# dselivanov/rsparse

Measured on AMD Instinct MI355X. Metric: als_iterations_per_sec, higher is better.
Workload: dtype f32 (Gram products of rows > 512 / <= 32 non-zeros as 2 x fp16 / 3 x bf16 split terms of the fp32 operands, fp32 accumulate; everything else fp32); 1 GPU; WRMF implicit ALS, CG(3), synthetic 10000000x1000000, 500155883 nnz, rank 128, lambda 0.1; survey_config=3, feedback=implicit, n_items=1000000, nnz=500155883, rank=128, solver=conjugate_gradient, cg_steps=3, parallelism=rows sharded x1, factors replicated

## Files before the change

rsparse_amd/build.py:

```python
import subprocess
import sys
import time
from concurrent.futures import ThreadPoolExecutor
from pathlib import Path

PKG = Path(__file__).resolve().parent
CSRC = PKG / "csrc"
SRC = [CSRC / n for n in ("wrmf_kernels.hip", "wrmf_cgq.hip", "wrmf_cgp.hip", "wrmf_ne.hip", "wrmf_chol.hip", "wrmf_chol_wave.hip", "wrmf_chol_mf.hip", "wrmf_cg_mf.hip", "wrmf_chol_lr.hip",
                          "wrmf_topk.hip", "wrmf_topk_large.hip", "wrmf_similar.hip", "wrmf_metrics.hip", "wrmf_hits.hip", "wrmf_lists.hip", "wrmf_diversity.hip", "wrmf_mmr.hip", "wrmf_ranks.hip", "wrmf_score.hip", "wrmf_candidates.hip", "wrmf_sample.hip", "wrmf_sample_weighted.hip", "wrmf_split.hip", "wrmf_explain.hip", "wrmf_init.hip", "wrmf_ingest.hip", "wrmf_nnls.hip", "wrmf_bias.hip", "wrmf_lu.hip",
                          "wrmf_f64.hip", "wrmf_wide.hip", "wrmf_wide_cg.hip", "wrmf_ctx_kernels.hip", "wrmf_schedule.cpp", "wrmf_capi.cpp", "wrmf_f64_capi.cpp", "wrmf_ctx.cpp")]
HEADERS = [CSRC / "wrmf_chol_mf.attrs.csv", CSRC / "wrmf_mf.h", CSRC / "wrmf_internal.h", CSRC / "wrmf_capi_common.h", CSRC / "wrmf_schedule.h", CSRC / "wrmf_device.h", CSRC / "wrmf_sample_team.h", CSRC / "wrmf_wave.h", CSRC / "wrmf_ldlt.h", CSRC / "wrmf_f64.h", PKG.parent / "include" / "rsparse_wrmf_hip.h"]
DEPS = SRC + HEADERS
OUT = PKG / "lib" / "librsparse_wrmf_hip.so"
FLAGS = ["--offload-arch=gfx950", "-O3", "-std=c++17", "-fPIC"]


EXTRA_FLAGS = {n: ["-mllvm", "-forceattrs-csv-path=" + str(CSRC / "wrmf_chol_mf.attrs.csv"), "-fno-slp-vectorize"] for n in ("wrmf_chol_mf.hip", "wrmf_cg_mf.hip")}
AUDITED = {"wrmf_chol_mf.hip", "wrmf_cg_mf.hip"}
REG_LIMIT = {"wrmf_cg_mf.hip": 512}
NO_SPILL = {"wrmf_cgq.hip": ("14als_cgq_kernelILi128ELi24ELi4ELi4E",),
            "wrmf_explain.hip": ("14explain_kernelIfLi128E",),
            "wrmf_sample.hip": ("13sample_kernelILi64E", "13sample_kernelILi256E"),
            "wrmf_sample_weighted.hip": ("22sample_weighted_kernelILi64E", "22sample_weighted_kernelILi256E"),
            "wrmf_hits.hip": ("18hit_metrics_kernelILb0E", "18hit_metrics_kernelILb1E"),
            "wrmf_lists.hip": ("19list_metrics_kernelILb0E", "19list_metrics_kernelILb1E"),
            "wrmf_diversity.hip": ("21list_diversity_kernelI", "21item_inv_norms_kernelI"),
            "wrmf_mmr.hip": ("10mmr_kernelI",),
            "wrmf_split.hip": ("split_count_wave_kernel", "split_count_team_kernel", "split_write_wave_kernel", "split_write_team_kernel")}
RESOURCE_FLAG = "-Rpass-analysis=kernel-resource-usage"


def resource_violations(remarks, patterns, limit=256):
    import re
    rows, cur = [], None
    for line in remarks.splitlines():
# ... 104 lines not shown
```

rsparse_amd/csrc/wrmf_capi.cpp:

```cpp
#include "../../include/rsparse_wrmf_hip.h"

#include <cxxabi.h>

#include <algorithm>
#include <cfloat>
#include <cmath>
#include <cstdlib>
#include <cstring>
#include <string>
#include <vector>

#include "wrmf_capi_common.h"

using namespace rsparse_hip;

struct rsparse_hip_csc {
  DevCSC d;
  int device = 0;
  std::vector<void*> owned;
};

namespace {
thread_local std::string g_err;
}
// ... 272 lines not shown
    if (we != hipSuccess) return hip_fail(we, wave_cg ? "launch_wide_cg_wave" : "launch_als_wide");
    if ((we = launch_sum_partials(g_ws.partials, wave_cg ? (size_t)grid_w : (size_t)grid, outw, s, g_ws.partials + g_ws.partial_slots())) != hipSuccess)
      return hip_fail(we, "launch_sum_partials");
    return RSPARSE_HIP_OK;
  }
  const bool cg = solver == RSPARSE_SOLVER_CONJUGATE_GRADIENT;
  const bool cgq = cg && use_cgq(rank, d_X, d_Y);
  QSchedule qs;
  qs.order = d.q_order;
  qs.cfg = d.q_cfg;
  qs.pair_first = d.q_pair_first;
  for (int b = 0; b < 7; b++) qs.off[b] = d.q_off[b];
  qs.team4_first = (implicit && bias && bias->gbias != 0.f) ? d.q_off[2] : d.q_team4_first;
  qs.team4_wide_first = (implicit && bias && bias->gbias != 0.f) ? d.q_off[2] : d.q_team4_wide_first;
  qs.pair_wide = cgp_wide_supported(rank, implicit, implicit && bias && bias->gbias != 0.f);
  const bool cg_mf = cgq && implicit && !bias && cg_mf_supported(rank, implicit) && d.q_order && d.q_off[1] > d.q_n_nec;
  if (cg_mf) {
    qs.mf_rows = d.q_order + d.q_n_nec;
    qs.mf_n = d.q_off[1] - d.q_n_nec;
  }
  const bool chol_mf = chol_mf_supported(rank) && !cg && solver == RSPARSE_SOLVER_CHOLESKY && !bias && d.q_order && ne_supported(rank) &&
                       use_cgq(rank, d_X, d_Y) && d.q_lr_first > d.q_off[1];
  const int mf_first = d.q_off[1];
  const int n_mf = chol_mf ? d.q_lr_first - mf_first : 0;
  const bool nec_lists = padded_rank(rank) > 64 && d.q_nec.wg > 0 && !chol_mf;
  const bool ne_chol = !cg && solver == RSPARSE_SOLVER_CHOLESKY && !bias && (nec_lists || d.q_ne.wg > 0 || chol_mf) &&
                       ne_supported(rank) && use_cgq(rank, d_X, d_Y);
  qs.ne = (cg_mf || (ne_chol && nec_lists)) ? d.q_nec : ((implicit && padded_rank(rank) == 128) ? d.q_ne : d.q_ne1);
  const size_t chol_base = chol2_loss_slots(d.n_cols);
  const size_t slots = cgq ? cgq_loss_slots(qs, rank, implicit) : (cg ? cg_loss_slots(d.n_cols, d.n_long)
// ... 1896 lines not shown
```

rsparse_amd/csrc/wrmf_cgp.hip:

```cpp
#include "wrmf_internal.h"
#include "wrmf_device.h"

namespace rsparse_hip {
namespace {

using namespace dev;

constexpr int kPairMaxSweeps = 4;

template <int NQ>
struct PairSmem {
  static constexpr int KP = 128, ps = KP + 8, os = KP + 4;
  static constexpr size_t gfrag = NQ == 16 ? (size_t)4 * 16 * 1024 : 0;
  static constexpr size_t nxt = NQ == 16 ? (size_t)4 * 2 * 2 * 64 * 4 : 0;
  static constexpr size_t bytes = gfrag + (size_t)2 * 8 * ps * 2 + (size_t)8 * os * 4 + (size_t)4 * 8 * NQ * 4 + nxt + 16;
};

template <bool GB, bool KFULL = false, int NQ = 8>
__global__ __launch_bounds__(256, 2) void als_cgp_kernel(AlsArgs a, const int32_t* __restrict__ rows, int n_rows, int iters,
                                                        size_t loss_slot0) {
  constexpr int KP = 128, RPN = 8, VW = 4, NV = 2;
  static_assert(NQ == 8 || (NQ == 16 && KFULL && !GB), "the 32-slot kernel: rank 128, no global bias");
  constexpr bool GREG = NQ == 8;
  using SM = PairSmem<NQ>;
  extern __shared__ __attribute__((aligned(16))) char smem[];
  char* sGf = smem + (size_t)(threadIdx.x >> 6) * 16 * 1024;
  _Float16* sPh = reinterpret_cast<_Float16*>(smem + SM::gfrag);
  _Float16* sPl = sPh + 8 * SM::ps;
  float* sOut = reinterpret_cast<float*>(sPl + 8 * SM::ps);
  float* sTsv = sOut + 8 * SM::os;
  float* sNx = sTsv + 4 * 8 * NQ + (threadIdx.x >> 6) * 256;
  const int tid = threadIdx.x, lane = tid & 63, wv = rfl(tid >> 6);
  const int g = lane >> 4, i = lane & 15, H = lane >> 5, g2 = g & 1;
  const int k = KFULL ? KP : a.k;
  const float gbias = GB ? a.gbias : 0.f, ltgt = GB ? a.loss_tgt_const : 1.f;
  for (int e = tid; e < 4 * 8 * NQ; e += 256) sTsv[e] = 0.f;
  f16x8 gAh[GREG ? 2 : 1][GREG ? 4 : 1], gAl[GREG ? 2 : 1][GREG ? 4 : 1];
  float ginv;
  {
    const int m = lane & 15, kb = lane >> 4;
    float gmax = 0.f;
#pragma unroll
    for (int t = 0; t < 2; t++)
#pragma unroll
      for (int ks = 0; ks < 4; ks++)
#pragma unroll
        for (int e = 0; e < 8; e++) {
          const int r = 32 * wv + 16 * t + m, c = 32 * ks + 8 * kb + e;
// ... 19 lines not shown
          const float g1v = a.XtX[(size_t)min(r, k - 1) * k + min(c + 1, k - 1)];
          const float g1 = g1v * ((r < k && c + 1 < k) ? 1.f : 0.f);
          split_f16(g0 * gs, g1 * gs, hi[e / 2], lo[e / 2]);
        }
        const uint4 h4 = {hi[0], hi[1], hi[2], hi[3]}, l4 = {lo[0], lo[1], lo[2], lo[3]};
        if constexpr (GREG) {
          gAh[t][ks] = __builtin_bit_cast(f16x8, h4);
          gAl[t][ks] = __builtin_bit_cast(f16x8, l4);
        } else {
          *reinterpret_cast<uint4*>(sGf + ((t * 4 + ks) * 2 + 0) * 1024 + lane * 16) = h4;
          *reinterpret_cast<uint4*>(sGf + ((t * 4 + ks) * 2 + 1) * 1024 + lane * 16) = l4;
        }
      }
  }
  __syncthreads();
  float* tacc = sTsv + wv * 8 * NQ + 2 * NQ * H;
  float* tcur = tacc + 4 * NQ;
  const int lslot = NQ == 16 ? i + 16 * g2 : i;
  const bool lgrp = NQ == 16 || g2 == 0;
  const int col = 2 * wv + H;
  double wloss = 0.0;
  const int wave_global = blockIdx.x * 4 + wv, total_waves = gridDim.x * 4;
  auto ridx = [&](const int itn) { return (wave_global + itn * total_waves) * 2 + H; };
  int row_c = 0, p1_c = 0, p2_c = 0, row_n = 0;
  if (iters > 0 && ridx(0) < n_rows) {
    row_c = rows[ridx(0)];
    p1_c = a.col_ptrs[row_c];
    p2_c = a.col_ptrs[row_c + 1];
  }
  if (iters > 1 && ridx(1) < n_rows) row_n = rows[ridx(1)];

  int idn[GREG ? NQ : 1];
  float cvn[GREG ? NQ : 1], cln = 0.f;
#pragma unroll
  for (int q = 0; q < (GREG ? NQ : 1); q++) {
    idn[q] = 0;
    cvn[q] = 0.f;
  }
  auto request_indices = [&](const bool valid, const int np1, const int ncnt, const int buf) {
    if constexpr (!GREG) {
      const int e = lane & 31;
      const bool in = valid && e < ncnt;
      float* slot = sNx + buf * 128;
      dma4(in ? static_cast<const void*>(a.row_idx + np1 + e) : static_cast<const void*>(a.zero_row), (unsigned)rfl((int)lds_addr(slot)));
      dma4(in ? static_cast<const void*>(a.vals + np1 + e) : static_cast<const void*>(a.zero_row), (unsigned)rfl((int)lds_addr(slot + 64)));
      return;
    }
#pragma unroll
    for (int q = 0; q < NQ; q++) {
      const int s = 2 * q + g2;
      const int j = (valid && s < ncnt) ? np1 + s : 0;
      idn[q] = a.row_idx[j];
      cvn[q] = a.vals[j];
    }
    cln = a.vals[(valid && lslot < ncnt) ? np1 + lslot : 0];
  };
// ... 21 lines not shown
      int p1_n = 0, p2_n = 0, row_nn = 0;
      if (it + 1 < iters && ridx(it + 1) < n_rows) {
        p1_n = a.col_ptrs[row_n];
        p2_n = a.col_ptrs[row_n + 1];
      }
      if (it + 2 < iters && ridx(it + 2) < n_rows) row_nn = rows[ridx(it + 2)];
      row_c = row_n;
      p1_c = p1_n;
      p2_c = p2_n;
      row_n = row_nn;
    }
    const int cnt = p2 - p1;
    float* yrow = a.Y + (size_t)row * k;
    const bool live = have && (GB || cnt > 0);
    if (have && !live) {
      for (int e = lane & 31; e < k; e += 32) yrow[e] = 0.f;
    }
    const int wcnt = max(__builtin_amdgcn_readlane(cnt, 0), __builtin_amdgcn_readlane(cnt, 32));
    auto blk_on = [&](const int q) { return q < 4 || wcnt > 2 * (q & ~3); };

    float x[RPN], r[RPN], p[RPN], ap[RPN];
    auto load_warm_start = [&]() {
#pragma unroll
      for (int b = 0; b < NV; b++) {
        const int off = b * 16 * VW + i * VW;
        float4 pc = make_float4(0.f, 0.f, 0.f, 0.f);
        if (have && off < k) pc = *reinterpret_cast<const float4*>(yrow + off);
        const float* pf = reinterpret_cast<const float*>(&pc);
#pragma unroll
        for (int c = 0; c < VW; c++) x[b * VW + c] = pf[c];
      }
    };
    if constexpr (KFULL) load_warm_start();
    float xt[NQ][RPN], cv[GREG ? NQ : 1];
    const float* nx = sNx + (it & 1) * 128 + 32 * H;
    {
      int id[NQ];
#pragma unroll
      for (int q = 0; q < NQ; q++) {
        if constexpr (!GREG) {
          id[q] = __float_as_int(nx[2 * q + g2]);
        } else if constexpr (KFULL) {
          id[q] = idn[q];
          cv[q] = cvn[q];
        } else {
          const int s = 2 * q + g2;
          const int j = s < cnt ? p1 + s : 0;
          id[q] = 0;
          cv[q] = 0.f;
          if (blk_on(q)) {
            id[q] = a.row_idx[j];
            cv[q] = a.vals[j];
          }
        }
      }
#pragma unroll
      for (int q = 0; q < NQ; q++) {
        const bool in = 2 * q + g2 < cnt;
        id[q] = in ? id[q] : 0;
        if constexpr (GREG) cv[q] = in ? cv[q] : 0.f;
      }
#pragma unroll
      for (int q = 0; q < NQ; q++) {
        const bool in = 2 * q + g2 < cnt;
        const float* src = in ? a.X + (size_t)id[q] * k : a.zero_row;
#pragma unroll
        for (int b = 0; b < NV; b++) {
          const int off = b * 16 * VW + i * VW;
          if constexpr (KFULL) {
            float4 pc = make_float4(0.f, 0.f, 0.f, 0.f);
            if (blk_on(q)) pc = *reinterpret_cast<const float4*>(src + off);
            const float* pf = reinterpret_cast<const float*>(&pc);
#pragma unroll
            for (int c = 0; c < VW; c++) xt[q][b * VW + c] = pf[c];
          } else {
            float4 pc = make_float4(0.f, 0.f, 0.f, 0.f);
            if (blk_on(q)) pc = *reinterpret_cast<const float4*>(src + min(off, k - VW));
            const float* pf = reinterpret_cast<const float*>(&pc);
#pragma unroll
// ... 2 lines not shown
        }
      }
    }
    float cl;
    if constexpr (!GREG) cl = nx[64 + lslot];
    else if constexpr (KFULL) cl = (lgrp && lslot < cnt) ? cln : 0.f;
    else cl = (lgrp && lslot < cnt) ? a.vals[p1 + lslot] : 0.f;

    if constexpr (!KFULL) load_warm_start();

    auto sweep = [&](const float(&v)[RPN], const int mode, float(&out)[RPN], float& loss_out) {
      float acc[RPN];
#pragma unroll
      for (int rr = 0; rr < RPN; rr++) acc[rr] = 0.f;
      float vinv = 0.f;
      if (mode != 2) {
        float vmax = 0.f;
#pragma unroll
        for (int rr = 0; rr < RPN; rr++) vmax = fmaxf(vmax, fabsf(v[rr]));
        vmax = row16_max(vmax);
        const int ve = fp16_scale_exp(vmax);
        const float vs = __uint_as_float((unsigned)ve << 23);
        vinv = __uint_as_float((unsigned)(254 - ve) << 23) * (mode == 0 ? -1.f : 1.f);
        {
          float w4[VW];
#pragma unroll
          for (int c = 0; c < VW; c++) w4[c] = (g2 == 0 ? v[c] : v[VW + c]) * vs;
          unsigned h0, l0, h1, l1;
          split_f16(w4[0], w4[1], h0, l0);
          split_f16(w4[2], w4[3], h1, l1);
          const int off = col * SM::ps + g2 * 16 * VW + i * VW;
          *reinterpret_cast<uint2*>(sPh + off) = make_uint2(h0, h1);
          *reinterpret_cast<uint2*>(sPl + off) = make_uint2(l0, l1);
        }
        __syncthreads();
        f32x4 d0[2], d1[2];
#pragma unroll
        for (int t = 0; t < 2; t++) d0[t] = d1[t] = f32x4{0.f, 0.f, 0.f, 0.f};
        const int nb = (lane & 7) * SM::ps + 8 * (lane >> 4);
#pragma unroll
        for (int ks = 0; ks < 4; ks++) {
          const f16x8 bh = *reinterpret_cast<const f16x8*>(sPh + nb + 32 * ks);
          const f16x8 bl = *reinterpret_cast<const f16x8*>(sPl + nb + 32 * ks);
#pragma unroll
          for (int t = 0; t < 2; t++) {
            f16x8 ah, al;
            if constexpr (GREG) {
              ah = gAh[t][ks];
              al = gAl[t][ks];
            } else {
              ah = *reinterpret_cast<const f16x8*>(sGf + ((t * 4 + ks) * 2 + 0) * 1024 + lane * 16);
              al = *reinterpret_cast<const f16x8*>(sGf + ((t * 4 + ks) * 2 + 1) * 1024 + lane * 16);
            }
            d0[t] = __builtin_amdgcn_mfma_f32_16x16x32_f16(ah, bh, d0[t], 0, 0, 0);
            d1[t] = __builtin_amdgcn_mfma_f32_16x16x32_f16(ah, bl, d1[t], 0, 0, 0);
            d1[t] = __builtin_amdgcn_mfma_f32_16x16x32_f16(al, bh, d1[t], 0, 0, 0);
          }
        }
        if ((lane & 15) < 8) {
#pragma unroll
          for (int t = 0; t < 2; t++) {
            const f32x4 d = (d0[t] + d1[t]) * ginv;
            *reinterpret_cast<f32x4*>(sOut + (lane & 15) * SM::os + 32 * wv + 16 * t + 4 * (lane >> 4)) = d;
          }
        }
      }
      float lacc = 0.f;
      if (mode != 2) {
        float* trec = (mode == 0 ? tacc : tcur) + g2;
#pragma unroll
        for (int q0 = 0; q0 < NQ; q0 += 4) {
          if (blk_on(q0)) {
            float t[4];
            f32x2 s2[4];
#pragma unroll
            for (int u = 0; u < 4; u++) s2[u] = f32x2{0.f, 0.f};
#pragma unroll
            for (int rr = 0; rr < RPN; rr += 2) {
              const f32x2 va = {v[rr], v[rr + 1]};
#pragma unroll
              for (int u = 0; u < 4; u++) {
                const f32x2 xa = {xt[q0 + u][rr], xt[q0 + u][rr + 1]};
                s2[u] = __builtin_elementwise_fma(xa, va, s2[u]);
              }
            }
#pragma unroll
            for (int u = 0; u < 4; u++) t[u] = s2[u].x + s2[u].y;
#pragma unroll
            for (int u = 0; u < 4; u++) t[u] += dpp<0xB1>(t[u]);
#pragma unroll
            for (int u = 0; u < 4; u++) t[u] += dpp<0x4E>(t[u]);
#pragma unroll
            for (int u = 0; u < 4; u++) t[u] += dpp<0x141>(t[u]);
#pragma unroll
            for (int u = 0; u < 4; u++) t[u] += dpp<0x140>(t[u]);
#pragma unroll
            for (int u = 0; u < 4; u++) {
              const int q = q0 + u;
              const float c = GREG ? cv[q] : nx[64 + 2 * q + g2];
              trec[2 * q] = t[u];
              const float w = mode == 0 ? c - (c - 1.f) * (GB ? t[u] + gbias : t[u]) : (c - 1.f) * t[u];
#pragma unroll
              for (int rr = 0; rr < RPN; rr++) acc[rr] = fmaf(w, xt[q][rr], acc[rr]);
            }
          }
        }
      } else {
        wave_sync();
        const float t = tacc[lslot];
        const float dd = ltgt - t;
        lacc = pair_sum(row16_sum((lgrp && lslot < cnt) ? cl * dd * dd : 0.f));
      }
      if (mode != 2) {
        __syncthreads();
        const float f = g2 == 0 ? vinv : 0.f;
#pragma unroll
        for (int b = 0; b < NV; b++) {
          const f32x4 o = *reinterpret_cast<const f32x4*>(sOut + col * SM::os + b * 16 * VW + i * VW);
#pragma unroll
          for (int c = 0; c < VW; c++) acc[b * VW + c] = fmaf(f, o[c], acc[b * VW + c]);
        }
#pragma unroll
        for (int rr = 0; rr < RPN; rr++) out[rr] = pair_sum(acc[rr]);
        if constexpr (GB) {
          if (mode == 0) {
#pragma unroll
            for (int b = 0; b < NV; b++) {
              const int off = b * 16 * VW + i * VW;
              const float4 pc = *reinterpret_cast<const float4*>(a.rhs_init + min(off, k - VW));
              const float* pf = reinterpret_cast<const float*>(&pc);
#pragma unroll
              for (int c = 0; c < VW; c++) out[b * VW + c] += off < k ? pf[c] : 0.f;
            }
          }
        }
      } else {
        loss_out = lacc;
      }
// ... 33 lines not shown
          const float beta = (float)((double)rsnew / (double)rsold);
#pragma unroll
          for (int rr = 0; rr < RPN; rr++) p[rr] = fmaf(p[rr], beta, r[rr]);
          rsold = rsnew;
        }
      }
    }
    float rl = 0.f;
    sweep(x, 2, ap, rl);
    if constexpr (KFULL) {
      settle_indices();
    }
    if (live) {
      const float xx = dot16(x, x);
      wloss += (double)rl + a.lambda_loss * (double)xx;
      if (g2 == 0) {
#pragma unroll
        for (int b = 0; b < NV; b++) {
          const int off = b * 16 * VW + i * VW;
          if (off < k) {
            float4 pc;
            float* pf = reinterpret_cast<float*>(&pc);
#pragma unroll
            for (int c = 0; c < VW; c++) pf[c] = x[b * VW + c];
            *reinterpret_cast<float4*>(yrow + off) = pc;
          }
        }
      }
    }
  }
  const double other = __shfl(wloss, 32);
  if (lane == 0) a.loss_partials[loss_slot0 + (size_t)blockIdx.x * 4 + wv] = wloss + other;
}

}

bool cgp_supported(int k, bool implicit) { return implicit && k > 64 && k <= 128 && k % 4 == 0; }
bool cgp_wide_supported(int k, bool implicit, bool gbias) { return implicit && k == 128 && !gbias; }

int cgp_grid(int n_rows) {
  if (n_rows <= 0) return 0;
  const long pairs = ((long)n_rows + 1) / 2;
  long per_wave = 32;
  const long spread = 4L * 512;
  if (pairs < spread * per_wave) per_wave = (pairs + spread - 1) / spread;
  if (per_wave < 1) per_wave = 1;
  return (int)((pairs + 4 * per_wave - 1) / (4 * per_wave));
}

hipError_t launch_als_cgp(const AlsArgs& a, const int32_t* rows, int n_rows, bool wide, size_t loss_slot0, hipStream_t s,
                          hipEvent_t* ev_slot) {
  const int grid = cgp_grid(n_rows);
  if (grid <= 0) return hipSuccess;
  const long pairs = ((long)n_rows + 1) / 2;
  const int iters = (int)((pairs + (long)grid * 4 - 1) / ((long)grid * 4));
  const bool gb = a.gbias != 0.f;
  const bool full = !gb && a.k == 128;
  if (wide && !full) return hipErrorInvalidValue;
  auto k0 = als_cgp_kernel<false, false>;
  auto k0f = als_cgp_kernel<false, true>;
  auto k1 = als_cgp_kernel<true, false>;
  auto kw = als_cgp_kernel<false, true, 16>;
  const void* fn = wide ? reinterpret_cast<const void*>(kw)
                        : gb ? reinterpret_cast<const void*>(k1) : (full ? reinterpret_cast<const void*>(k0f) : reinterpret_cast<const void*>(k0));
  const size_t lds = wide ? PairSmem<16>::bytes : PairSmem<8>::bytes;
  hipError_t err = hipFuncSetAttribute(fn, hipFuncAttributeMaxDynamicSharedMemorySize, (int)lds);
  if (err != hipSuccess) return err;
  prof_note(ev_slot, fn);
  if (wide) hipLaunchKernelGGL(kw, dim3(grid), dim3(256), lds, s, a, rows, n_rows, iters, loss_slot0);
  else if (gb) hipLaunchKernelGGL(k1, dim3(grid), dim3(256), lds, s, a, rows, n_rows, iters, loss_slot0);
  else if (full) hipLaunchKernelGGL(k0f, dim3(grid), dim3(256), lds, s, a, rows, n_rows, iters, loss_slot0);
  else hipLaunchKernelGGL(k0, dim3(grid), dim3(256), lds, s, a, rows, n_rows, iters, loss_slot0);
  return hipGetLastError();
}

}
```

rsparse_amd/csrc/wrmf_cgq.hip:

```cpp
#include <algorithm>

#include "wrmf_internal.h"
#include "wrmf_device.h"

namespace rsparse_hip {
namespace {

using namespace dev;

constexpr int kGvFirstMinCapq = 16;
constexpr int kStreamPrefixQ = 4;
constexpr int kIdxPrefetchMaxWpr = 2;

constexpr int kMaxSavedSweeps = 4;

template <int KP>
struct QG {
  static constexpr int RPN = KP / 16;
  static constexpr int VW = RPN >= 4 ? 4 : RPN;
  static constexpr int NV = RPN / VW;
  __device__ static __forceinline__ int elem(int i, int r) { return (r / VW) * (16 * VW) + i * VW + (r % VW); }
};

template <int VW>
struct Piece;
template <>
struct Piece<4> { using type = float4; };
template <>
struct Piece<2> { using type = float2; };

__device__ __forceinline__ float groups_reduce_scatter4(const float a0, const float a1, const float a2, const float a3) {
  const auto s01 = __builtin_amdgcn_permlane16_swap(__float_as_uint(a0), __float_as_uint(a1), false, false);
  const float c = __uint_as_float(s01[0]) + __uint_as_float(s01[1]);
  const auto s23 = __builtin_amdgcn_permlane16_swap(__float_as_uint(a2), __float_as_uint(a3), false, false);
  const float d = __uint_as_float(s23[0]) + __uint_as_float(s23[1]);
  const auto t = __builtin_amdgcn_permlane32_swap(__float_as_uint(c), __float_as_uint(d), false, false);
  return __uint_as_float(t[0]) + __uint_as_float(t[1]);
}
template <bool ON>
__device__ __forceinline__ int opaque_lane(int l) {
  if constexpr (ON) asm volatile("" : "+v"(l));
  return l;
}
template <int KP, int CAPQ, int WAVES, int WPR, int STREAM, bool IMPLICIT, int DMF = 0>
struct QSmem {
  static constexpr size_t gram_floats = (IMPLICIT && DMF != 1) ? (size_t)KP * KP : 0;
  static constexpr size_t vec_floats = IMPLICIT ? (size_t)WAVES * KP : 0;
  static constexpr size_t red_floats = WPR > 1 ? (size_t)2 * WAVES * KP + 2 * WAVES : 0;
  static constexpr bool cv_lds = !STREAM && CAPQ * (KP / 16) > 128;
  static constexpr bool wideq = !STREAM && CAPQ * (KP / 16) > 160;
  static constexpr size_t tsv_floats = (STREAM && !IMPLICIT) ? 0 : (size_t)WAVES * (cv_lds ? 3 : 2) * CAPQ * 4;
  static constexpr size_t pre_floats = STREAM ? (size_t)WAVES * kStreamPrefixQ * 4 * KP : 0;
  static constexpr int dmf_ps = KP + 8, dmf_os = KP + 4;
  static constexpr size_t dmf_floats = DMF ? (size_t)WAVES * dmf_ps + (size_t)WAVES * dmf_os : 0;
  static constexpr size_t pfx_floats =
      (!STREAM && WPR > kIdxPrefetchMaxWpr && (CAPQ == 16 || CAPQ == 20 || CAPQ == 24)) ? (size_t)WAVES * 2 * CAPQ * 4 : 0;
  static constexpr size_t wl_floats = cv_lds ? (size_t)WAVES * 2 : 0;
// ... 917 lines not shown
int concurrent_buckets() { return g_launch_mode; }

size_t bucket_slots(const QSchedule& q, int b, int k, bool implicit) {
  const int cfg = cfg_of_kp(padded_rank(k));
  const BucketDef d = kBuckets[cfg][b];
  if (d.wpr <= 0) return 0;
  if (d.stream && ne_supported(k)) return (size_t)(q.ne.entries + q.ne.nsplit) + (size_t)(q.mf_n > 0 ? cg_mf_loss_slots(q.mf_n) : 0);
  const int rows = q.off[b + 1] - q.off[b];
  if (b == 1 && padded_rank(k) == 128) {
    const int wide = team4_wide_first(q), split = team4_first(q);
    return (size_t)cgq_bucket_grid(wide - q.off[b], b, cfg) * d.waves + (size_t)cgq_team4_wide_grid(split - wide) * kTeam4Waves +
           (size_t)cgq_team4_grid(q.off[b + 1] - split) * kTeam4Waves;
  }
  if (b == kNB - 1 && rows > 0 && cgp_supported(k, implicit)) {
    const int split = std::min(std::max(q.pair_first, q.off[b]), q.off[b + 1]);
    const size_t main = q.pair_wide ? (size_t)cgp_grid(split - q.off[b]) * 4 : (size_t)cgq_bucket_grid(split - q.off[b], b, cfg) * d.waves;
    return main + (size_t)cgp_grid(q.off[b + 1] - split) * 4;
  }
  return (size_t)cgq_bucket_grid(rows, b, cfg) * d.waves;
}

template <int KP, int CFG, bool IMPLICIT, bool GB>
hipError_t launch_all(const AlsArgs& a, const QSchedule& q, hipStream_t s, hipEvent_t* ev) {
  hipError_t err;
  size_t slot = 0;
  const int cmode = ev ? 0 : concurrent_buckets();
  const bool overlap = cmode != 0;
  bool forked = false;
  if (overlap) {
    if ((err = g_bs.ensure()) != hipSuccess) return err;
  }
#define RSP_BUCKET(B)                                                                                       \
// ... 49 lines not shown
          const int g_main = cgq_bucket_grid(n_main, B, CFG), g_w4 = cgq_team4_wide_grid(n_w4);             \
          if ((err = launch_bucket<KP, D.waves, D.capq, D.wpr, D.stream, IMPLICIT, GB>(a, q.order + first, n_main, g_main, slot, \
                                                                                  bs, ev ? ev + B : nullptr)) != hipSuccess) \
            return err;                                                                                     \
          if ((err = launch_bucket<KP, kTeam4Waves, kTeam4WideCapq, kTeam4Waves, 0, IMPLICIT, GB>(          \
                   a, q.order + wide, n_w4, g_w4, slot + (size_t)g_main * D.waves, bs,                      \
                   n_main > 0 ? nullptr : (ev ? ev + B : nullptr))) != hipSuccess)                          \
            return err;                                                                                     \
          if ((err = launch_bucket<KP, kTeam4Waves, kTeam4Capq, kTeam4Waves, 0, IMPLICIT, GB>(              \
                   a, q.order + split, n_t4, cgq_team4_grid(n_t4),                                          \
                   slot + (size_t)g_main * D.waves + (size_t)g_w4 * kTeam4Waves, bs,                        \
                   n_main + n_w4 > 0 ? nullptr : (ev ? ev + B : nullptr))) != hipSuccess)                   \
            return err;                                                                                     \
        } else if (B == kNB - 1 && cgp_supported(a.k, IMPLICIT)) {                    \
           \
                                                 \
          const int first = q.off[B], split = std::min(std::max(q.pair_first, first), q.off[B + 1]);         \
          const int n_main = split - first, n_pair = q.off[B + 1] - split;                                   \
          size_t main_slots;                                                                                \
          if (q.pair_wide) {                                                                                \
            if ((err = launch_als_cgp(a, q.order + first, n_main, true, slot, bs, ev ? ev + B : nullptr)) != hipSuccess) \
              return err;                                                                                   \
            main_slots = (size_t)cgp_grid(n_main) * 4;                                                      \
          } else {                                                                                          \
            const int g_main = cgq_bucket_grid(n_main, B, CFG);                                             \
            if ((err = launch_bucket<KP, D.waves, D.capq, D.wpr, D.stream, IMPLICIT, GB>(a, q.order + first, n_main, g_main, slot, \
                                                                                    bs, ev ? ev + B : nullptr)) != hipSuccess) \
              return err;                                                                                   \
            main_slots = (size_t)g_main * D.waves;                                                          \
          }                                                                                                 \
          if ((err = launch_als_cgp(a, q.order + split, n_pair, false, slot + main_slots, bs,               \
                                    n_main > 0 ? nullptr : (ev ? ev + B : nullptr))) != hipSuccess)           \
            return err;                                                                                     \
        } else if ((err = launch_bucket<KP, D.waves, D.capq, D.wpr, D.stream, IMPLICIT, GB>(a, q.order + q.off[B], n, grid, slot, \
                                                                                bs, ev ? ev + B : nullptr)) != hipSuccess) \
          return err;                                                                                       \
        if (side) {                                                                                         \
          if ((err = hipEventRecord(g_bs.done[B], bs)) != hipSuccess) return err;                           \
          if ((err = hipStreamWaitEvent(s, g_bs.done[B], 0)) != hipSuccess) return err;                     \
        }                                                                                                   \
      }                                                                                                     \
      slot += bucket_slots(q, B, a.k, IMPLICIT);                                                             \
    }                                                                                                       \
  }
  RSP_BUCKET(0)
  RSP_BUCKET(1)
// ... 73 lines not shown
```

rsparse_amd/csrc/wrmf_internal.h:

```cpp
#pragma once
#include <hip/hip_runtime.h>
#include <cstdint>
#include <string>

#include "wrmf_schedule.h"

namespace rsparse_hip {

constexpr float kCgTol = 1e-10f;
constexpr double kCgTolD = 1e-10;
constexpr int kScdMaxIter = 10000;
constexpr float kScdTol = 1e-4f;
constexpr double kScdTolD = 1e-4;
constexpr float kNnlsEps = 1e-16f;
constexpr double kNnlsEpsD = 1e-16;

struct NeListSet {
  const int32_t* rows = nullptr;
  const int32_t* ptr = nullptr;
  int wg = 0;
  int entries = 0;
  const int32_t* segs = nullptr;
  int nseg = 0;
  const int32_t* split_rows = nullptr;
// ... 83 lines not shown
  int* ne_seg_flags;
  int ne_chol;
  int ne_chol_min;
  const unsigned* ne_stats;
  const float* mf_XtX;
  const unsigned* wave_stats;
};

struct QSchedule {
  const int32_t* order;
  int off[7];
  int pair_first;
  int team4_first;
  int team4_wide_first;
  bool pair_wide;
  int cfg;
  NeListSet ne;
  const int32_t* mf_rows = nullptr;
  int mf_n = 0;
};
int cgq_default_cfg();
void cgq_set_launch_mode(int mode);
int cgq_num_buckets();
int cgq_bucket_wpr(int cfg, int b);
int cgq_bucket_capq(int cfg, int b);
int cgq_bucket_waves(int cfg, int b);
int cgq_bucket_stream(int cfg, int b);
int cgq_bucket_grid(int n_rows, int bucket, int cfg);
int cgq_team4_grid(int n_rows);
int cgq_team4_wide_grid(int n_rows);
int cgq_bucket_of(int len, int cfg);
size_t cgq_loss_slots(const QSchedule& q, int k, bool implicit);
bool cgp_supported(int k, bool implicit);
bool cgp_wide_supported(int k, bool implicit, bool gbias);
int cgp_grid(int n_rows);
hipError_t launch_als_cgp(const AlsArgs& a, const int32_t* rows, int n_rows, bool wide, size_t loss_slot0, hipStream_t s,
                          hipEvent_t* ev_slot);
bool ne_supported(int k);
constexpr int kNeMinLen = 512;
constexpr int kNeSegFloats = 4 * (11 * 16 * 64 + 128 + 2);
hipError_t launch_ne_stats(const float* X, int64_t nx, const float* vals, int64_t nnz, unsigned* stats, hipStream_t s,
                           const float* absmax_hint = nullptr, const unsigned* cached_vstats = nullptr,
                           unsigned* save_vstats = nullptr);
hipError_t launch_als_ne(const AlsArgs& a, const QSchedule& q, bool implicit, double* row_loss, hipStream_t s,
                         hipEvent_t* ev_slot = nullptr);
hipError_t launch_gb_row_terms(const AlsArgs& a, const int32_t* rows, int n, float* out, int32_t* slot_of_row, hipStream_t s);
hipError_t launch_als_cgq(const AlsArgs& a, const QSchedule& q, bool implicit, hipStream_t s, hipEvent_t* ev = nullptr);

constexpr int kWavesPerWG = 4;
constexpr int kRowsPerWGShort = 64;
constexpr int kRowsPerWGLong = 8;
// ... 265 lines not shown
```

rsparse_amd/csrc/wrmf_schedule.cpp:

```cpp
#include "wrmf_schedule.h"

#include <algorithm>
#include <functional>
#include <queue>
#include <utility>

namespace rsparse_hip {

namespace {
int ne_slots(int cus) { return 2 * std::max(cus, 1); }
}

NeCut ne_cut(const int32_t* order, const int32_t* col_ptrs, int n_prefix, int64_t fixed, int cus) {
  NeCut c;
  if (n_prefix <= 0) return c;
  auto len_of = [&](int r) { return (int64_t)(col_ptrs[order[r] + 1] - col_ptrs[order[r]]); };
  auto steps_of = [](int64_t len) { return (len + 15) / 16; };
  const int n_slots = ne_slots(cus);
  int64_t total = 0;
  for (int r = 0; r < n_prefix; r++) total += steps_of(len_of(r)) + fixed;
  const int64_t share = std::max<int64_t>(1, total / n_slots);
  c.items.reserve((size_t)n_prefix + 64);
  int n_seg = 0;
  for (int r = 0; r < n_prefix; r++) {
    const int64_t len = len_of(r);
    const int64_t st = steps_of(len);
// ... 110 lines not shown
```

rsparse_amd/csrc/wrmf_schedule.h:

```cpp
#pragma once
#include <cstdint>
#include <vector>

namespace rsparse_hip {

constexpr int kTileNnz = 32;
constexpr int kTeam4Max = 320;
constexpr int kTeam4WideMax = 384;
constexpr int kCholLrMax = 64;
constexpr int kCholLongLen = 4096;
constexpr int kCgMfMax = 16384;
constexpr int kNeMaxSeg = 16;
constexpr int kNeMaxSegTotal = 1024;

struct NeCut {
  struct Item { int64_t cost; int32_t entry; };
  std::vector<Item> items;
  std::vector<int32_t> segs;
  std::vector<int32_t> split_rows;
  std::vector<int32_t> split_ptr;
  int nseg() const { return (int)(segs.size() / 6); }
};
struct NeDeal {
  std::vector<int32_t> rows, ptr;
  int wg() const { return ptr.empty() ? 0 : (int)ptr.size() - 1; }
};

NeCut ne_cut(const int32_t* order, const int32_t* col_ptrs, int n_prefix, int64_t fixed, int cus);
// ... 27 lines not shown
```

rsparse_amd/csrc/wrmf_wave.h:

```cpp
#pragma once
#include <hip/hip_runtime.h>

#include <type_traits>
#include <utility>

namespace rsparse_hip {
namespace dev {

typedef unsigned long long u64;
typedef float f32x2 __attribute__((ext_vector_type(2)));
typedef float f32x4 __attribute__((ext_vector_type(4)));
typedef float f32x16 __attribute__((ext_vector_type(16)));
typedef double f64x4 __attribute__((ext_vector_type(4)));
typedef _Float16 f16x2 __attribute__((ext_vector_type(2)));
typedef _Float16 f16x8 __attribute__((ext_vector_type(8)));
typedef __bf16 bf16x2 __attribute__((ext_vector_type(2)));
typedef __bf16 bf16x8 __attribute__((ext_vector_type(8)));
typedef unsigned u32x4 __attribute__((ext_vector_type(4)));

template <class F, int... I>
__device__ __forceinline__ void static_for_seq(F&& f, std::integer_sequence<int, I...>) {
  (f(std::integral_constant<int, I>{}), ...);
}
template <int N, class F>
__device__ __forceinline__ void static_for(F&& f) {
  static_for_seq(f, std::make_integer_sequence<int, N>{});
}

__device__ __forceinline__ void wave_sync() {
  __builtin_amdgcn_fence(__ATOMIC_RELEASE, "wavefront");
  __builtin_amdgcn_wave_barrier();
  __builtin_amdgcn_fence(__ATOMIC_ACQUIRE, "wavefront");
}

__device__ __forceinline__ float readlane_f(float v, int l) {
  return __int_as_float(__builtin_amdgcn_readlane(__float_as_int(v), l));
}
__device__ __forceinline__ int rfl(int v) { return __builtin_amdgcn_readfirstlane(v); }

__device__ __forceinline__ unsigned lds_addr(const void* p) {
  return (unsigned)(reinterpret_cast<uintptr_t>(p));
}
__device__ __forceinline__ void dma4(const void* g, unsigned lds_base) {
  asm volatile("s_mov_b32 m0, %1\n\ts_nop 0\n\tglobal_load_lds_dword %0, off" : : "v"(g), "s"(lds_base) : "memory", "m0");
}
__device__ __forceinline__ void dma16(const void* g, unsigned lds_base) {
  asm volatile("s_mov_b32 m0, %1\n\ts_nop 0\n\tglobal_load_lds_dwordx4 %0, off" : : "v"(g), "s"(lds_base) : "memory", "m0");
}
template <int N>
__device__ __forceinline__ void wait_vm() {
  asm volatile("s_waitcnt vmcnt(%0)" ::"n"(N) : "memory");
}

// ... 142 lines not shown
```

Measured before the change: 8.564 iterations/s.

## Add four-rows-per-wave CG pair kernel for short rows at rank 128

Adds a QUAD variant of the pair CG kernel in which each wave handles four short rows (16 lanes each, 16 slots per row) instead of two. The fp16 hi/lo panel and the output buffer share one LDS region, and the scheduler selects this variant for the short-row tail when rank is 128 with no global bias. The grid, visit count and loss-slot math are generalised to rows-per-wave. The aim is to use more of each wave on rows with few non-zeros, at the cost of an extra workgroup barrier and register-held B fragments per CG step.

```diff
diff --git a/rsparse_amd/build.py b/rsparse_amd/build.py
--- a/rsparse_amd/build.py
+++ b/rsparse_amd/build.py
@@ -19,6 +19,7 @@
 AUDITED = {"wrmf_chol_mf.hip", "wrmf_cg_mf.hip"}
 REG_LIMIT = {"wrmf_cg_mf.hip": 512}
 NO_SPILL = {"wrmf_cgq.hip": ("14als_cgq_kernelILi128ELi24ELi4ELi4E",),
+            "wrmf_cgp.hip": ("14als_cgp_kernelILb0ELb1ELi16ELb1E",),
             "wrmf_explain.hip": ("14explain_kernelIfLi128E",),
             "wrmf_sample.hip": ("13sample_kernelILi64E", "13sample_kernelILi256E"),
             "wrmf_sample_weighted.hip": ("22sample_weighted_kernelILi64E", "22sample_weighted_kernelILi256E"),
diff --git a/rsparse_amd/csrc/wrmf_capi.cpp b/rsparse_amd/csrc/wrmf_capi.cpp
--- a/rsparse_amd/csrc/wrmf_capi.cpp
+++ b/rsparse_amd/csrc/wrmf_capi.cpp
@@ -310,6 +310,7 @@
   qs.team4_first = (implicit && bias && bias->gbias != 0.f) ? d.q_off[2] : d.q_team4_first;
   qs.team4_wide_first = (implicit && bias && bias->gbias != 0.f) ? d.q_off[2] : d.q_team4_wide_first;
   qs.pair_wide = cgp_wide_supported(rank, implicit, implicit && bias && bias->gbias != 0.f);
+  qs.pair_quad = cgp_quad_supported(rank, implicit, implicit && bias && bias->gbias != 0.f);
   const bool cg_mf = cgq && implicit && !bias && cg_mf_supported(rank, implicit) && d.q_order && d.q_off[1] > d.q_n_nec;
   if (cg_mf) {
     qs.mf_rows = d.q_order + d.q_n_nec;
diff --git a/rsparse_amd/csrc/wrmf_cgp.hip b/rsparse_amd/csrc/wrmf_cgp.hip
--- a/rsparse_amd/csrc/wrmf_cgp.hip
+++ b/rsparse_amd/csrc/wrmf_cgp.hip
@@ -8,30 +8,40 @@
 
 constexpr int kPairMaxSweeps = 4;
 
-template <int NQ>
+template <int NQ, bool QUAD = false>
 struct PairSmem {
-  static constexpr int KP = 128, ps = KP + 8, os = KP + 4;
+  static constexpr int KP = 128, ps = KP + 8, os = QUAD ? KP + 8 : KP + 4;
+  static constexpr int cols = QUAD ? 16 : 8;
+  static constexpr int pcs = QUAD ? 2 * ps : ps;
   static constexpr size_t gfrag = NQ == 16 ? (size_t)4 * 16 * 1024 : 0;
   static constexpr size_t nxt = NQ == 16 ? (size_t)4 * 2 * 2 * 64 * 4 : 0;
-  static constexpr size_t bytes = gfrag + (size_t)2 * 8 * ps * 2 + (size_t)8 * os * 4 + (size_t)4 * 8 * NQ * 4 + nxt + 16;
+  static constexpr size_t pub = (size_t)2 * cols * ps * 2, out = (size_t)cols * os * 4;
+  static_assert(!QUAD || (pub == out && (size_t)pcs * 2 == (size_t)os * 4), "QUAD: one column, one stretch of LDS");
+  static constexpr size_t bytes = gfrag + (QUAD ? pub : pub + out) + (size_t)4 * 8 * NQ * 4 + nxt + 16;
 };
-
-template <bool GB, bool KFULL = false, int NQ = 8>
+static_assert(PairSmem<16>::bytes <= 81920 && PairSmem<16, true>::bytes <= 81920, "two workgroups per CU");
+
+template <bool GB, bool KFULL = false, int NQ = 8, bool QUAD = false>
 __global__ __launch_bounds__(256, 2) void als_cgp_kernel(AlsArgs a, const int32_t* __restrict__ rows, int n_rows, int iters,
                                                         size_t loss_slot0) {
   constexpr int KP = 128, RPN = 8, VW = 4, NV = 2;
   static_assert(NQ == 8 || (NQ == 16 && KFULL && !GB), "the 32-slot kernel: rank 128, no global bias");
+  static_assert(!QUAD || NQ == 16, "four rows per wave: 16 slots per group, G in LDS");
   constexpr bool GREG = NQ == 8;
-  using SM = PairSmem<NQ>;
+  constexpr int RW = QUAD ? 4 : 2, GL = 64 / RW;
+  constexpr int SS = QUAD ? 1 : 2;
+  using SM = PairSmem<NQ, QUAD>;
   extern __shared__ __attribute__((aligned(16))) char smem[];
   char* sGf = smem + (size_t)(threadIdx.x >> 6) * 16 * 1024;
   _Float16* sPh = reinterpret_cast<_Float16*>(smem + SM::gfrag);
-  _Float16* sPl = sPh + 8 * SM::ps;
-  float* sOut = reinterpret_cast<float*>(sPl + 8 * SM::ps);
-  float* sTsv = sOut + 8 * SM::os;
+  _Float16* sPl = QUAD ? sPh + SM::ps : sPh + 8 * SM::ps;
+  float* sOut = QUAD ? reinterpret_cast<float*>(sPh) : reinterpret_cast<float*>(sPl + 8 * SM::ps);
+  float* sTsv = QUAD ? reinterpret_cast<float*>(sPh + 16 * SM::pcs) : sOut + 8 * SM::os;
   float* sNx = sTsv + 4 * 8 * NQ + (threadIdx.x >> 6) * 256;
   const int tid = threadIdx.x, lane = tid & 63, wv = rfl(tid >> 6);
   const int g = lane >> 4, i = lane & 15, H = lane >> 5, g2 = g & 1;
+  const int R = QUAD ? g : H;
+  const int gs = QUAD ? 0 : g2;
   const int k = KFULL ? KP : a.k;
   const float gbias = GB ? a.gbias : 0.f, ltgt = GB ? a.loss_tgt_const : 1.f;
   for (int e = tid; e < 4 * 8 * NQ; e += 256) sTsv[e] = 0.f;
@@ -81,14 +91,14 @@
       }
   }
   __syncthreads();
-  float* tacc = sTsv + wv * 8 * NQ + 2 * NQ * H;
+  float* tacc = sTsv + wv * 8 * NQ + (QUAD ? NQ * g : 2 * NQ * H);
   float* tcur = tacc + 4 * NQ;
-  const int lslot = NQ == 16 ? i + 16 * g2 : i;
+  const int lslot = (NQ == 16 && !QUAD) ? i + 16 * g2 : i;
   const bool lgrp = NQ == 16 || g2 == 0;
-  const int col = 2 * wv + H;
+  const int col = RW * wv + R;
   double wloss = 0.0;
   const int wave_global = blockIdx.x * 4 + wv, total_waves = gridDim.x * 4;
-  auto ridx = [&](const int itn) { return (wave_global + itn * total_waves) * 2 + H; };
+  auto ridx = [&](const int itn) { return (wave_global + itn * total_waves) * RW + R; };
   int row_c = 0, p1_c = 0, p2_c = 0, row_n = 0;
   if (iters > 0 && ridx(0) < n_rows) {
     row_c = rows[ridx(0)];
@@ -106,7 +116,7 @@
   }
   auto request_indices = [&](const bool valid, const int np1, const int ncnt, const int buf) {
     if constexpr (!GREG) {
-      const int e = lane & 31;
+      const int e = lane & (GL - 1);
       const bool in = valid && e < ncnt;
       float* slot = sNx + buf * 128;
       dma4(in ? static_cast<const void*>(a.row_idx + np1 + e) : static_cast<const void*>(a.zero_row), (unsigned)rfl((int)lds_addr(slot)));
@@ -158,10 +168,16 @@
     float* yrow = a.Y + (size_t)row * k;
     const bool live = have && (GB || cnt > 0);
     if (have && !live) {
-      for (int e = lane & 31; e < k; e += 32) yrow[e] = 0.f;
-    }
-    const int wcnt = max(__builtin_amdgcn_readlane(cnt, 0), __builtin_amdgcn_readlane(cnt, 32));
-    auto blk_on = [&](const int q) { return q < 4 || wcnt > 2 * (q & ~3); };
+      if constexpr (QUAD) {
+#pragma unroll
+        for (int b = 0; b < NV; b++) *reinterpret_cast<float4*>(yrow + b * 16 * VW + i * VW) = make_float4(0.f, 0.f, 0.f, 0.f);
+      } else {
+        for (int e = lane & 31; e < k; e += 32) yrow[e] = 0.f;
+      }
+    }
+    int wcnt = max(__builtin_amdgcn_readlane(cnt, 0), __builtin_amdgcn_readlane(cnt, 32));
+    if constexpr (QUAD) wcnt = max(wcnt, max(__builtin_amdgcn_readlane(cnt, 16), __builtin_amdgcn_readlane(cnt, 48)));
+    auto blk_on = [&](const int q) { return q < 4 || wcnt > SS * (q & ~3); };
 
     float x[RPN], r[RPN], p[RPN], ap[RPN];
     auto load_warm_start = [&]() {
@@ -177,13 +193,13 @@
     };
     if constexpr (KFULL) load_warm_start();
     float xt[NQ][RPN], cv[GREG ? NQ : 1];
-    const float* nx = sNx + (it & 1) * 128 + 32 * H;
+    const float* nx = sNx + (it & 1) * 128 + (QUAD ? 16 * g : 32 * H);
     {
       int id[NQ];
 #pragma unroll
       for (int q = 0; q < NQ; q++) {
         if constexpr (!GREG) {
-          id[q] = __float_as_int(nx[2 * q + g2]);
+          id[q] = __float_as_int(QUAD ? nx[q] : nx[2 * q + g2]);
         } else if constexpr (KFULL) {
           id[q] = idn[q];
           cv[q] = cvn[q];
@@ -200,13 +216,13 @@
       }
 #pragma unroll
       for (int q = 0; q < NQ; q++) {
-        const bool in = 2 * q + g2 < cnt;
+        const bool in = SS * q + gs < cnt;
         id[q] = in ? id[q] : 0;
         if constexpr (GREG) cv[q] = in ? cv[q] : 0.f;
       }
 #pragma unroll
       for (int q = 0; q < NQ; q++) {
-        const bool in = 2 * q + g2 < cnt;
+        const bool in = SS * q + gs < cnt;
         const float* src = in ? a.X + (size_t)id[q] * k : a.zero_row;
 #pragma unroll
         for (int b = 0; b < NV; b++) {
@@ -239,6 +255,8 @@
 #pragma unroll
       for (int rr = 0; rr < RPN; rr++) acc[rr] = 0.f;
       float vinv = 0.f;
+      const int ln = opaque_lane<QUAD>(lane), li = ln & 15, lg = ln >> 4;
+      const int lcol = QUAD ? RW * wv + lg : col;
       if (mode != 2) {
         float vmax = 0.f;
 #pragma unroll
@@ -247,7 +265,18 @@
         const int ve = fp16_scale_exp(vmax);
         const float vs = __uint_as_float((unsigned)ve << 23);
         vinv = __uint_as_float((unsigned)(254 - ve) << 23) * (mode == 0 ? -1.f : 1.f);
-        {
+        if constexpr (QUAD) {
+          wave_sync();
+#pragma unroll
+          for (int b = 0; b < NV; b++) {
+            unsigned h0, l0, h1, l1;
+            split_f16(v[b * VW] * vs, v[b * VW + 1] * vs, h0, l0);
+            split_f16(v[b * VW + 2] * vs, v[b * VW + 3] * vs, h1, l1);
+            const int off = lcol * SM::pcs + b * 16 * VW + li * VW;
+            *reinterpret_cast<uint2*>(sPh + off) = make_uint2(h0, h1);
+            *reinterpret_cast<uint2*>(sPl + off) = make_uint2(l0, l1);
+          }
+        } else {
           float w4[VW];
 #pragma unroll
           for (int c = 0; c < VW; c++) w4[c] = (g2 == 0 ? v[c] : v[VW + c]) * vs;
@@ -262,11 +291,26 @@
         f32x4 d0[2], d1[2];
 #pragma unroll
         for (int t = 0; t < 2; t++) d0[t] = d1[t] = f32x4{0.f, 0.f, 0.f, 0.f};
-        const int nb = (lane & 7) * SM::ps + 8 * (lane >> 4);
+        const int nb = QUAD ? li * SM::pcs + 8 * lg : (lane & 7) * SM::ps + 8 * (lane >> 4);
+        f16x8 bhs[QUAD ? 4 : 1], bls[QUAD ? 4 : 1];
+        if constexpr (QUAD) {
+#pragma unroll
+          for (int ks = 0; ks < 4; ks++) {
+            bhs[ks] = *reinterpret_cast<const f16x8*>(sPh + nb + 32 * ks);
+            bls[ks] = *reinterpret_cast<const f16x8*>(sPl + nb + 32 * ks);
+          }
+          __syncthreads();
+        }
 #pragma unroll
         for (int ks = 0; ks < 4; ks++) {
-          const f16x8 bh = *reinterpret_cast<const f16x8*>(sPh + nb + 32 * ks);
-          const f16x8 bl = *reinterpret_cast<const f16x8*>(sPl + nb + 32 * ks);
+          f16x8 bh, bl;
+          if constexpr (QUAD) {
+            bh = bhs[ks];
+            bl = bls[ks];
+          } else {
+            bh = *reinterpret_cast<const f16x8*>(sPh + nb + 32 * ks);
+            bl = *reinterpret_cast<const f16x8*>(sPl + nb + 32 * ks);
+          }
 #pragma unroll
           for (int t = 0; t < 2; t++) {
             f16x8 ah, al;
@@ -274,25 +318,26 @@
               ah = gAh[t][ks];
               al = gAl[t][ks];
             } else {
-              ah = *reinterpret_cast<const f16x8*>(sGf + ((t * 4 + ks) * 2 + 0) * 1024 + lane * 16);
-              al = *reinterpret_cast<const f16x8*>(sGf + ((t * 4 + ks) * 2 + 1) * 1024 + lane * 16);
+              ah = *reinterpret_cast<const f16x8*>(sGf + ((t * 4 + ks) * 2 + 0) * 1024 + (QUAD ? ln : lane) * 16);
+              al = *reinterpret_cast<const f16x8*>(sGf + ((t * 4 + ks) * 2 + 1) * 1024 + (QUAD ? ln : lane) * 16);
             }
             d0[t] = __builtin_amdgcn_mfma_f32_16x16x32_f16(ah, bh, d0[t], 0, 0, 0);
             d1[t] = __builtin_amdgcn_mfma_f32_16x16x32_f16(ah, bl, d1[t], 0, 0, 0);
             d1[t] = __builtin_amdgcn_mfma_f32_16x16x32_f16(al, bh, d1[t], 0, 0, 0);
           }
         }
-        if ((lane & 15) < 8) {
+        if (QUAD || (lane & 15) < 8) {
 #pragma unroll
           for (int t = 0; t < 2; t++) {
             const f32x4 d = (d0[t] + d1[t]) * ginv;
-            *reinterpret_cast<f32x4*>(sOut + (lane & 15) * SM::os + 32 * wv + 16 * t + 4 * (lane >> 4)) = d;
+            float* po = QUAD ? sOut + li * SM::os + 32 * wv + 16 * t + 4 * lg : sOut + (lane & 15) * SM::os + 32 * wv + 16 * t + 4 * (lane >> 4);
+            *reinterpret_cast<f32x4*>(po) = d;
           }
         }
       }
       float lacc = 0.f;
       if (mode != 2) {
-        float* trec = (mode == 0 ? tacc : tcur) + g2;
+        float* trec = (mode == 0 ? tacc : tcur) + gs;
 #pragma unroll
         for (int q0 = 0; q0 < NQ; q0 += 4) {
           if (blk_on(q0)) {
@@ -322,8 +367,8 @@
 #pragma unroll
             for (int u = 0; u < 4; u++) {
               const int q = q0 + u;
-              const float c = GREG ? cv[q] : nx[64 + 2 * q + g2];
-              trec[2 * q] = t[u];
+              const float c = GREG ? cv[q] : (QUAD ? nx[64 + q] : nx[64 + 2 * q + g2]);
+              trec[SS * q] = t[u];
               const float w = mode == 0 ? c - (c - 1.f) * (GB ? t[u] + gbias : t[u]) : (c - 1.f) * t[u];
 #pragma unroll
               for (int rr = 0; rr < RPN; rr++) acc[rr] = fmaf(w, xt[q][rr], acc[rr]);
@@ -334,19 +379,21 @@
         wave_sync();
         const float t = tacc[lslot];
         const float dd = ltgt - t;
-        lacc = pair_sum(row16_sum((lgrp && lslot < cnt) ? cl * dd * dd : 0.f));
+        const float ls = row16_sum((lgrp && lslot < cnt) ? cl * dd * dd : 0.f);
+        lacc = QUAD ? ls : pair_sum(ls);
       }
       if (mode != 2) {
         __syncthreads();
-        const float f = g2 == 0 ? vinv : 0.f;
+        const float f = (QUAD || g2 == 0) ? vinv : 0.f;
 #pragma unroll
         for (int b = 0; b < NV; b++) {
-          const f32x4 o = *reinterpret_cast<const f32x4*>(sOut + col * SM::os + b * 16 * VW + i * VW);
+          const float* po = QUAD ? sOut + lcol * SM::os + b * 16 * VW + li * VW : sOut + col * SM::os + b * 16 * VW + i * VW;
+          const f32x4 o = *reinterpret_cast<const f32x4*>(po);
 #pragma unroll
           for (int c = 0; c < VW; c++) acc[b * VW + c] = fmaf(f, o[c], acc[b * VW + c]);
         }
 #pragma unroll
-        for (int rr = 0; rr < RPN; rr++) out[rr] = pair_sum(acc[rr]);
+        for (int rr = 0; rr < RPN; rr++) out[rr] = QUAD ? acc[rr] : pair_sum(acc[rr]);
         if constexpr (GB) {
           if (mode == 0) {
 #pragma unroll
@@ -410,7 +457,7 @@
     if (live) {
       const float xx = dot16(x, x);
       wloss += (double)rl + a.lambda_loss * (double)xx;
-      if (g2 == 0) {
+      if (QUAD || g2 == 0) {
 #pragma unroll
         for (int b = 0; b < NV; b++) {
           const int off = b * 16 * VW + i * VW;
@@ -426,44 +473,43 @@
     }
   }
   const double other = __shfl(wloss, 32);
-  if (lane == 0) a.loss_partials[loss_slot0 + (size_t)blockIdx.x * 4 + wv] = wloss + other;
+  if constexpr (QUAD) {
+    const double wsum = (wloss + __shfl(wloss, 16)) + (other + __shfl(wloss, 48));
+    if (lane == 0) a.loss_partials[loss_slot0 + (size_t)blockIdx.x * 4 + wv] = wsum;
+  } else {
+    if (lane == 0) a.loss_partials[loss_slot0 + (size_t)blockIdx.x * 4 + wv] = wloss + other;
+  }
 }
 
 }
 
 bool cgp_supported(int k, bool implicit) { return implicit && k > 64 && k <= 128 && k % 4 == 0; }
 bool cgp_wide_supported(int k, bool implicit, bool gbias) { return implicit && k == 128 && !gbias; }
-
-int cgp_grid(int n_rows) {
-  if (n_rows <= 0) return 0;
-  const long pairs = ((long)n_rows + 1) / 2;
-  long per_wave = 32;
-  const long spread = 4L * 512;
-  if (pairs < spread * per_wave) per_wave = (pairs + spread - 1) / spread;
-  if (per_wave < 1) per_wave = 1;
-  return (int)((pairs + 4 * per_wave - 1) / (4 * per_wave));
-}
-
-hipError_t launch_als_cgp(const AlsArgs& a, const int32_t* rows, int n_rows, bool wide, size_t loss_slot0, hipStream_t s,
+bool cgp_quad_supported(int k, bool implicit, bool gbias) { return implicit && k == 128 && !gbias; }
+
+hipError_t launch_als_cgp(const AlsArgs& a, const int32_t* rows, int n_rows, CgpForm form, size_t loss_slot0, hipStream_t s,
                           hipEvent_t* ev_slot) {
-  const int grid = cgp_grid(n_rows);
+  const int rpw = cgp_rows_per_wave(form);
+  const int grid = cgp_grid(n_rows, rpw);
   if (grid <= 0) return hipSuccess;
-  const long pairs = ((long)n_rows + 1) / 2;
-  const int iters = (int)((pairs + (long)grid * 4 - 1) / ((long)grid * 4));
+  const int iters = cgp_visits(n_rows, rpw);
   const bool gb = a.gbias != 0.f;
   const bool full = !gb && a.k == 128;
-  if (wide && !full) return hipErrorInvalidValue;
+  const bool wide = form == kCgpWide, quad = form == kCgpQuad;
+  if ((wide || quad) && !full) return hipErrorInvalidValue;
   auto k0 = als_cgp_kernel<false, false>;
   auto k0f = als_cgp_kernel<false, true>;
   auto k1 = als_cgp_kernel<true, false>;
   auto kw = als_cgp_kernel<false, true, 16>;
-  const void* fn = wide ? reinterpret_cast<const void*>(kw)
+  auto kq = als_cgp_kernel<false, true, 16, true>;
+  const void* fn = quad ? reinterpret_cast<const void*>(kq) : wide ? reinterpret_cast<const void*>(kw)
                         : gb ? reinterpret_cast<const void*>(k1) : (full ? reinterpret_cast<const void*>(k0f) : reinterpret_cast<const void*>(k0));
-  const size_t lds = wide ? PairSmem<16>::bytes : PairSmem<8>::bytes;
+  const size_t lds = quad ? PairSmem<16, true>::bytes : wide ? PairSmem<16>::bytes : PairSmem<8>::bytes;
   hipError_t err = hipFuncSetAttribute(fn, hipFuncAttributeMaxDynamicSharedMemorySize, (int)lds);
   if (err != hipSuccess) return err;
   prof_note(ev_slot, fn);
-  if (wide) hipLaunchKernelGGL(kw, dim3(grid), dim3(256), lds, s, a, rows, n_rows, iters, loss_slot0);
+  if (quad) hipLaunchKernelGGL(kq, dim3(grid), dim3(256), lds, s, a, rows, n_rows, iters, loss_slot0);
+  else if (wide) hipLaunchKernelGGL(kw, dim3(grid), dim3(256), lds, s, a, rows, n_rows, iters, loss_slot0);
   else if (gb) hipLaunchKernelGGL(k1, dim3(grid), dim3(256), lds, s, a, rows, n_rows, iters, loss_slot0);
   else if (full) hipLaunchKernelGGL(k0f, dim3(grid), dim3(256), lds, s, a, rows, n_rows, iters, loss_slot0);
   else hipLaunchKernelGGL(k0, dim3(grid), dim3(256), lds, s, a, rows, n_rows, iters, loss_slot0);
diff --git a/rsparse_amd/csrc/wrmf_cgq.hip b/rsparse_amd/csrc/wrmf_cgq.hip
--- a/rsparse_amd/csrc/wrmf_cgq.hip
+++ b/rsparse_amd/csrc/wrmf_cgq.hip
@@ -36,11 +36,6 @@
   const float d = __uint_as_float(s23[0]) + __uint_as_float(s23[1]);
   const auto t = __builtin_amdgcn_permlane32_swap(__float_as_uint(c), __float_as_uint(d), false, false);
   return __uint_as_float(t[0]) + __uint_as_float(t[1]);
-}
-template <bool ON>
-__device__ __forceinline__ int opaque_lane(int l) {
-  if constexpr (ON) asm volatile("" : "+v"(l));
-  return l;
 }
 template <int KP, int CAPQ, int WAVES, int WPR, int STREAM, bool IMPLICIT, int DMF = 0>
 struct QSmem {
@@ -988,8 +983,9 @@
   }
   if (b == kNB - 1 && rows > 0 && cgp_supported(k, implicit)) {
     const int split = std::min(std::max(q.pair_first, q.off[b]), q.off[b + 1]);
-    const size_t main = q.pair_wide ? (size_t)cgp_grid(split - q.off[b]) * 4 : (size_t)cgq_bucket_grid(split - q.off[b], b, cfg) * d.waves;
-    return main + (size_t)cgp_grid(q.off[b + 1] - split) * 4;
+    const size_t main = q.pair_wide ? (size_t)cgp_loss_slots(split - q.off[b], cgp_rows_per_wave(kCgpWide))
+                                    : (size_t)cgq_bucket_grid(split - q.off[b], b, cfg) * d.waves;
+    return main + (size_t)cgp_loss_slots(q.off[b + 1] - split, cgp_rows_per_wave(q.pair_quad ? kCgpQuad : kCgpPair));
   }
   return (size_t)cgq_bucket_grid(rows, b, cfg) * d.waves;
 }
@@ -1069,14 +1065,14 @@
             return err;                                                                                     \
         } else if (B == kNB - 1 && cgp_supported(a.k, IMPLICIT)) {                    \
            \
-                                                 \
+                  \
           const int first = q.off[B], split = std::min(std::max(q.pair_first, first), q.off[B + 1]);         \
           const int n_main = split - first, n_pair = q.off[B + 1] - split;                                   \
           size_t main_slots;                                                                                \
           if (q.pair_wide) {                                                                                \
-            if ((err = launch_als_cgp(a, q.order + first, n_main, true, slot, bs, ev ? ev + B : nullptr)) != hipSuccess) \
+            if ((err = launch_als_cgp(a, q.order + first, n_main, kCgpWide, slot, bs, ev ? ev + B : nullptr)) != hipSuccess) \
               return err;                                                                                   \
-            main_slots = (size_t)cgp_grid(n_main) * 4;                                                      \
+            main_slots = (size_t)cgp_loss_slots(n_main, cgp_rows_per_wave(kCgpWide));                       \
           } else {                                                                                          \
             const int g_main = cgq_bucket_grid(n_main, B, CFG);                                             \
             if ((err = launch_bucket<KP, D.waves, D.capq, D.wpr, D.stream, IMPLICIT, GB>(a, q.order + first, n_main, g_main, slot, \
@@ -1084,7 +1080,7 @@
               return err;                                                                                   \
             main_slots = (size_t)g_main * D.waves;                                                          \
           }                                                                                                 \
-          if ((err = launch_als_cgp(a, q.order + split, n_pair, false, slot + main_slots, bs,               \
+          if ((err = launch_als_cgp(a, q.order + split, n_pair, q.pair_quad ? kCgpQuad : kCgpPair, slot + main_slots, bs, \
                                     n_main > 0 ? nullptr : (ev ? ev + B : nullptr))) != hipSuccess)           \
             return err;                                                                                     \
         } else if ((err = launch_bucket<KP, D.waves, D.capq, D.wpr, D.stream, IMPLICIT, GB>(a, q.order + q.off[B], n, grid, slot, \
diff --git a/rsparse_amd/csrc/wrmf_internal.h b/rsparse_amd/csrc/wrmf_internal.h
--- a/rsparse_amd/csrc/wrmf_internal.h
+++ b/rsparse_amd/csrc/wrmf_internal.h
@@ -121,6 +121,7 @@
   int team4_first;
   int team4_wide_first;
   bool pair_wide;
+  bool pair_quad = false;
   int cfg;
   NeListSet ne;
   const int32_t* mf_rows = nullptr;
@@ -140,8 +141,10 @@
 size_t cgq_loss_slots(const QSchedule& q, int k, bool implicit);
 bool cgp_supported(int k, bool implicit);
 bool cgp_wide_supported(int k, bool implicit, bool gbias);
-int cgp_grid(int n_rows);
-hipError_t launch_als_cgp(const AlsArgs& a, const int32_t* rows, int n_rows, bool wide, size_t loss_slot0, hipStream_t s,
+bool cgp_quad_supported(int k, bool implicit, bool gbias);
+enum CgpForm { kCgpPair = 0, kCgpWide = 1, kCgpQuad = 2 };
+inline int cgp_rows_per_wave(CgpForm form) { return form == kCgpQuad ? 4 : 2; }
+hipError_t launch_als_cgp(const AlsArgs& a, const int32_t* rows, int n_rows, CgpForm form, size_t loss_slot0, hipStream_t s,
                           hipEvent_t* ev_slot);
 bool ne_supported(int k);
 constexpr int kNeMinLen = 512;
diff --git a/rsparse_amd/csrc/wrmf_schedule.cpp b/rsparse_amd/csrc/wrmf_schedule.cpp
--- a/rsparse_amd/csrc/wrmf_schedule.cpp
+++ b/rsparse_amd/csrc/wrmf_schedule.cpp
@@ -10,6 +10,23 @@
 namespace {
 int ne_slots(int cus) { return 2 * std::max(cus, 1); }
 }
+
+int cgp_grid(int n_rows, int rows_per_wave) {
+  if (n_rows <= 0) return 0;
+  const long sets = ((long)n_rows + rows_per_wave - 1) / rows_per_wave;
+  long per_wave = 32;
+  const long spread = 4L * 512;
+  if (sets < spread * per_wave) per_wave = (sets + spread - 1) / spread;
+  if (per_wave < 1) per_wave = 1;
+  return (int)((sets + 4 * per_wave - 1) / (4 * per_wave));
+}
+int cgp_visits(int n_rows, int rows_per_wave) {
+  const long grid = cgp_grid(n_rows, rows_per_wave);
+  if (grid <= 0) return 0;
+  const long sets = ((long)n_rows + rows_per_wave - 1) / rows_per_wave;
+  return (int)((sets + grid * 4 - 1) / (grid * 4));
+}
+int64_t cgp_loss_slots(int n_rows, int rows_per_wave) { return (int64_t)cgp_grid(n_rows, rows_per_wave) * 4; }
 
 NeCut ne_cut(const int32_t* order, const int32_t* col_ptrs, int n_prefix, int64_t fixed, int cus) {
   NeCut c;
diff --git a/rsparse_amd/csrc/wrmf_schedule.h b/rsparse_amd/csrc/wrmf_schedule.h
--- a/rsparse_amd/csrc/wrmf_schedule.h
+++ b/rsparse_amd/csrc/wrmf_schedule.h
@@ -12,6 +12,10 @@
 constexpr int kCgMfMax = 16384;
 constexpr int kNeMaxSeg = 16;
 constexpr int kNeMaxSegTotal = 1024;
+
+int cgp_grid(int n_rows, int rows_per_wave = 2);
+int cgp_visits(int n_rows, int rows_per_wave = 2);
+int64_t cgp_loss_slots(int n_rows, int rows_per_wave = 2);
 
 struct NeCut {
   struct Item { int64_t cost; int32_t entry; };
diff --git a/rsparse_amd/csrc/wrmf_wave.h b/rsparse_amd/csrc/wrmf_wave.h
--- a/rsparse_amd/csrc/wrmf_wave.h
+++ b/rsparse_amd/csrc/wrmf_wave.h
@@ -37,6 +37,12 @@
   return __int_as_float(__builtin_amdgcn_readlane(__float_as_int(v), l));
 }
 __device__ __forceinline__ int rfl(int v) { return __builtin_amdgcn_readfirstlane(v); }
+
+template <bool ON>
+__device__ __forceinline__ int opaque_lane(int l) {
+  if constexpr (ON) asm volatile("" : "+v"(l));
+  return l;
+}
 
 __device__ __forceinline__ unsigned lds_addr(const void* p) {
   return (unsigned)(reinterpret_cast<uintptr_t>(p));
```

Measured after the change: 8.668 iterations/s, median of 6. +1.2%, better.
